# eora-ai/torchok

Measured on AMD Instinct MI355X. Metric: images/sec (node) ResNet-50 224px bs256/GPU; step p50 ms, higher is better.
Workload: dtype bf16

## Files before the change

### include/tok.h

```cpp
#ifndef TOK_H_
#define TOK_H_

#include <stddef.h>
#include <stdint.h>

#ifdef __cplusplus
extern "C" {
#endif

typedef enum tok_status {
  TOK_OK = 0,
  TOK_ERR_INVALID = -1,
  TOK_ERR_LAUNCH = -2,
  TOK_ERR_WORKSPACE = -3
} tok_status;

typedef enum tok_dtype { TOK_F32 = 0, TOK_F16 = 1, TOK_BF16 = 2 } tok_dtype;

typedef struct tok_conv_desc {
  int32_t n, h, w, c;
  int32_t k;
  int32_t r, s;
  int32_t p, q;
  int32_t stride, pad;
// ... 49 lines not shown
int tok_relu_mask_reduce(const void* dout, const uint8_t* mask, int64_t m, int c, void* dz, float* partial, void* stream);
int tok_bn3_bwd_prepare(const float* G, const float* w, const float* wz, const float* zsum, const float* partial, int rows,
                        int64_t count, int p, int k, const float* gamma, const float* mean, const float* rstd,
                        float* dgamma, float* dbeta, int param_accumulate, float* coef, float* dw, int dw_accumulate,
                        void* wa, void* wb, float* cvec, float* ws ,
                        void* stream);
size_t tok_bn3_bwd_prepare_ws_floats(int p, int k);
int tok_conv_dgrad_bias(const tok_conv_desc* d, const void* dy, const void* w_dgrad, const float* bias, void* dx,
                        int accumulate, const void* bn_y, const uint8_t* bn_mask, float* partial, void* stream);
int tok_subsample2_fwd(const void* x, int n, int h, int w, int c, void* out, void* stream);
int tok_subsample2_bwd(const void* dsub, int n, int h, int w, int c, void* dx, int accumulate, void* stream);
int tok_conv_dgrad_subacc_ok(const tok_conv_desc* d);
int tok_conv_dgrad_subacc(const tok_conv_desc* d, const void* dy, const void* w_dgrad, void* dx, const void* dsub,
                          const void* bn_y , const uint8_t* mask ,
                          float* partial , int mask_store, void* stream);
int tok_conv_dgrad2_ok(const tok_conv_desc* d1, const tok_conv_desc* d2);
int tok_conv_dgrad2(const tok_conv_desc* d1, const void* dy1, const void* w1_dgrad, const tok_conv_desc* d2, const void* dy2,
                    const void* w2_dgrad, const float* bias , void* dx, int accumulate,
                    const void* bn_y , const uint8_t* bn_mask , float* partial ,
                    void* stream);
size_t tok_conv_wgrad_ws_bytes(const tok_conv_desc* d);
int tok_conv_wgrad(const tok_conv_desc* d, const void* x, const void* dy, float* dw,
                   int k_real, int c_real, void* ws, size_t ws_bytes, int accumulate,
                   void* stream);
int tok_conv_wgrad_bias_ok(const tok_conv_desc* d);
size_t tok_conv_wgrad_bias_ws_bytes(const tok_conv_desc* d);
int tok_conv_wgrad_bias(const tok_conv_desc* d, const void* x, const void* dy, float* dw, int k_real, int c_real,
                        void* ws, size_t ws_bytes, int accumulate, float* dbias, int bias_accumulate, void* stream);


// ... 361 lines not shown
```

### torchok_amd/_C.py

```python
import ctypes
import os
from ctypes import POINTER, Structure, c_char_p, c_float, c_int, c_int32, c_int64, c_size_t, c_void_p

_HERE = os.path.dirname(os.path.abspath(__file__))
LIB_PATH = os.environ.get('TOK_LIB') or os.path.join(_HERE, 'lib', 'libtok_gfx950.so')

TOK_F32, TOK_F16, TOK_BF16 = 0, 1, 2
TOK_CE_LOSS_FLOATS = 2050


class ConvDesc(Structure):
    _fields_ = [('n', c_int32), ('h', c_int32), ('w', c_int32), ('c', c_int32),
                ('k', c_int32), ('r', c_int32), ('s', c_int32),
                ('p', c_int32), ('q', c_int32),
                ('stride', c_int32), ('pad', c_int32), ('s_pad', c_int32)]


class PackItem(Structure):
    _fields_ = [('src', c_void_p), ('dst_fwd', c_void_p), ('dst_dgrad', c_void_p),
                ('k', c_int32), ('r', c_int32), ('s', c_int32), ('c', c_int32),
                ('k_pad', c_int32), ('s_pad', c_int32), ('c_pad', c_int32), ('block_start', c_int32)]


TOK_GRAD_CLIP_MAX_PARTIALS = 1024
# ... 55 lines not shown
    'tok_colsum': (c_int, [_P, c_int64, c_int, c_int, _P, c_int, _P]),
    'tok_bn_gram_finalize': (c_int, [_P, _P, _P, c_int64, c_int, c_int, _P, _P, _P, _P, _P, c_float, c_float, _P, _P, _P, _P, _P, _P]),
    'tok_conv_fwd_bn_apply': (c_int, [POINTER(ConvDesc), _P, _P, _P, _P, _P, c_int, _P, _P, _P]),
    'tok_conv_dgrad_maskstore': (c_int, [POINTER(ConvDesc), _P, _P, _P, c_int, _P, _P, _P]),
    'tok_relu_mask_reduce': (c_int, [_P, _P, c_int64, c_int, _P, _P, _P]),
    'tok_bn3_bwd_prepare': (c_int, [_P, _P, _P, _P, _P, c_int, c_int64, c_int, c_int, _P, _P, _P, _P, _P, c_int, _P, _P, c_int,
                                    _P, _P, _P, _P, _P]),
    'tok_bn3_bwd_prepare_ws_floats': (c_size_t, [c_int, c_int]),
    'tok_conv_dgrad_bias': (c_int, [POINTER(ConvDesc), _P, _P, _P, _P, c_int, _P, _P, _P, _P]),
    'tok_conv_dgrad2_ok': (c_int, [POINTER(ConvDesc), POINTER(ConvDesc)]),
    'tok_conv_dgrad2': (c_int, [POINTER(ConvDesc), _P, _P, POINTER(ConvDesc), _P, _P, _P, _P, c_int, _P, _P, _P, _P]),
    'tok_subsample2_fwd': (c_int, [_P, c_int, c_int, c_int, c_int, _P, _P]),
    'tok_subsample2_bwd': (c_int, [_P, c_int, c_int, c_int, c_int, _P, c_int, _P]),
    'tok_conv_dgrad_subacc_ok': (c_int, [POINTER(ConvDesc)]),
    'tok_conv_dgrad_subacc': (c_int, [POINTER(ConvDesc), _P, _P, _P, _P, _P, _P, _P, c_int, _P]),
    'tok_softmax_ce_fwd': (c_int, [_P, _P, c_int, c_int, c_int, c_int64, _P, _P, _P, _P]),
    'tok_softmax_ce_bwd': (c_int, [_P, _P, _P, _P, _P, c_int, c_int, c_int, c_int64, _P, _P]),
    'tok_softmax_ce_smooth_fwd': (c_int, [_P, _P, c_int, c_int, c_int, c_int64, c_float, _P, _P, _P, _P]),
    'tok_softmax_ce_smooth_bwd': (c_int, [_P, _P, _P, _P, _P, c_int, c_int, c_int, c_int64, c_float, _P, _P]),
    'tok_upsample_ce_serves': (c_int, [c_int, c_int]),
    'tok_upsample_ce_fwd': (c_int, [_P, c_int, c_int, c_int, c_int, c_int, c_int, c_int, _P, c_int64, _P, _P, _P, _P]),
    'tok_upsample_ce_bwd': (c_int, [_P, c_int, c_int, c_int, c_int, c_int, c_int, c_int, _P, c_int64, _P, _P, _P, _P, c_int, _P]),
    'tok_dice_rows': (c_int, [c_int64]),
    'tok_dice_fwd': (c_int, [_P, _P, c_int64, c_int, c_int, c_int, c_float, c_float, c_int, _P, c_int, _P, _P, _P, _P]),
    'tok_dice_bwd': (c_int, [_P, _P, _P, _P, c_int64, c_int, c_int, c_int, _P, _P]),
    'tok_bce_logits_fwd': (c_int, [_P, _P, c_int64, c_int, c_int, c_float, c_int, _P, _P]),
    'tok_bce_logits_bwd': (c_int, [_P, _P, _P, _P, c_int64, c_int, c_int, c_float, c_int, _P, _P]),
    'tok_relevance_matrix_multilabel': (c_int, [_P, _P, c_int, c_int, c_int, _P, _P]),
    'tok_embed_reg_fwd': (c_int, [_P, c_int, c_int, c_int, c_int, _P, _P, _P]),
    'tok_embed_reg_bwd': (c_int, [_P, _P, _P, c_float, c_int, c_int, c_int, c_int, _P, _P]),
# ... 165 lines not shown
```

### torchok_amd/csrc/conv_common.h

```cpp
#pragma once
#include "tok_common.h"

struct FastDiv {
  uint32_t mul, shift;
};
static inline FastDiv make_fastdiv(uint32_t d) {
  FastDiv f;
  if (d <= 1) { f.mul = 0; f.shift = 0; return f; }
  uint32_t l = 0;
  while ((1ull << l) < d) ++l;
  f.mul = (uint32_t)((((1ull << 32) * ((1ull << l) - d)) / d) + 1);
  f.shift = l;
  return f;
}
__device__ __forceinline__ uint32_t fdiv(uint32_t n, FastDiv f) {
  return (uint32_t)(((uint64_t)__umulhi(n, f.mul) + n) >> f.shift);
}

struct ConvArgs {
  const bf16* x;
  const bf16* w;
  bf16* y;
  const float* bias;
  float* stats;
// ... 38 lines not shown
int conv_s2d_launch(ConvArgs& a, hipStream_t st);

bool gemm256_geometry(const ConvArgs& a);
bool gemm256_modes(const ConvArgs& a);
bool gemm256_serves(const ConvArgs& a);
int gemm256_rows(const ConvArgs& a);
void gemm256_tiles(const ConvArgs& a, int* gridM, int* gridN);
int gemm256_grid(int gridM, int gridN);
int gemm256_launch(ConvArgs& a, hipStream_t st);

bool stem_win_serves(const ConvArgs& a);
int stem_win_grid(const ConvArgs& a);
int stem_win_launch(ConvArgs& a, hipStream_t st);
bool stem_wgrad_serves(const tok_conv_desc* d);
int stem_wgrad_launch(const tok_conv_desc* d, const void* x, const void* dy, float* ws, int slabs, hipStream_t st);
```

### torchok_amd/csrc/conv_igemm.hip

```cpp
#include "conv_common.h"
#include "pw_gemm.h"
#include <stdlib.h>

namespace {

constexpr int BK = 64;
#ifdef TOK_NO_FRAG_ASM
constexpr bool FRAG_ASM = false;
#else
constexpr bool FRAG_ASM = true;
#endif
#ifdef TOK_NO_DMA
constexpr bool DMA_ENABLED = false;
#else
constexpr bool DMA_ENABLED = true;
#endif

__device__ __forceinline__ int fw_swz(int n) {
  return ((0x78 >> (((n >> 3) & 3) << 1)) & 3) | (((n >> 1) & 1) << 2);
}

template <int BM, int BN, int IN_DIV, bool C4, int PWM>
__global__ __launch_bounds__(256, (BN == 64 && PWM != 4) ? 3 : 2) void conv_igemm_kernel(ConvArgs a) {
  constexpr bool PW = PWM != 0;
// ... 691 lines not shown
  if (c4 && !m.bnep && stem_win_serves(a)) {
    r.kernel = K_STEM_WIN;
    r.grid = stem_win_grid(a);
    if (m.stats && r.grid > r.stat_rows) r.grid = r.stat_rows;
  }
  return r;
}

ConvRoute route_dgrad(const tok_conv_desc* d, const ConvArgs& a, ConvMode m) {
  if (d->stride == 1 && conv_win_serves(a)) return route_window(K_WIN, a);
  if (d->stride == 2 && conv_s2d_serves(a, d->stride, d->pad)) return route_window(K_S2D, a);
  const bool pointwise = d->r == 1 && d->s == 1 && d->stride == 1 && d->pad == 0;
  return route_gemm(a, pointwise, pick_bn(d->c, a.Ktot, d->h == 1 && d->w == 1), m);
}

int launch_ring(const ConvArgs& a, const ConvRoute& r, hipStream_t st) {
  PwArgs p = {};
  p.x = a.x; p.w = a.w; p.y = a.y; p.bias = a.bias; p.stats = a.stats;
  p.stat_rows = r.stat_rows;
  p.e1 = a.accumulate ? a.y : a.ep_short;
  p.e2 = a.bn_y; p.mask_in = a.bn_mask; p.mask_out = a.ep_mask;
  p.ep_scale = a.ep_scale; p.ep_shift = a.ep_shift; p.ep_relu = a.ep_relu;
  p.accumulate = a.accumulate; p.mask_store = a.mask_store;
  if (a.sub != nullptr) { p.e1 = a.sub; p.accumulate = 1; p.e1_sub = 1; p.sub_H = a.P; p.sub_W = a.Q; }
  p.M = a.M; p.C = a.C; p.N = a.K; p.gridM = r.gridM; p.gridN = r.gridN;
  return pw_ring_launch(p, r.bn_tile, r.grid, st);
}

template <int BN>
int launch_igemm(ConvArgs& a, int pw, int in_div, bool c4, hipStream_t st) {
  if (pw == 1) return launch_pw<128, BN, 1, false, 1>(a, st);
  if (pw == 3) return launch_pw<128, BN, 1, false, 3>(a, st);
  if (pw == 4) return launch_pw<128, BN, 1, false, 4>(a, st);
  if (c4) return launch_pw<128, BN, 1, true, 0>(a, st);
  return in_div == 2 ? launch_pw<128, BN, 2, false, 0>(a, st) : launch_pw<128, BN, 1, false, 0>(a, st);
}

int run_route(ConvArgs& a, const ConvRoute& r, int in_div, bool c4, hipStream_t st) {
  a.gridM = r.gridM; a.gridN = r.gridN; a.grid = r.grid; a.stat_rows = r.stat_rows;
  if (a.stats != nullptr) {
    const bool rows_agree = r.kernel == K_GEMM256 ? r.gridM <= r.stat_rows
// ... 218 lines not shown
  if (dgrad_fill(d, a)) return 0;
  return route_dgrad(d, a, ConvMode{false, false,  true, false}).kernel == K_RING ? 1 : 0;
}

extern "C" int tok_conv_dgrad_subacc(const tok_conv_desc* d, const void* dy, const void* w_dgrad, void* dx, const void* dsub,
                                     const void* bn_y, const uint8_t* mask, float* partial, int mask_store, void* stream) {
  TOK_CHECK_ARG(dsub != nullptr, "tok_conv_dgrad_subacc: dsub must not be null");
  TOK_CHECK_ARG(!mask_store || (mask && partial && !bn_y), "tok_conv_dgrad_subacc: mask_store needs mask + partial, no bn_y");
  TOK_CHECK_ARG(mask_store || ((bn_y == nullptr) == (partial == nullptr)), "tok_conv_dgrad_subacc: bn_y and partial go together");
  DgradEpilogue ep = {}; ep.bn_y = bn_y; ep.bn_mask = mask; ep.partial = partial; ep.mask_store = mask_store; ep.sub = dsub;
  return dgrad_impl(d, dy, w_dgrad, dx, ep, stream, "tok_conv_dgrad_subacc");
}


namespace {
bool dgrad2_route(const tok_conv_desc* d1, const tok_conv_desc* d2, ConvRoute* r) {
  if (d1 == nullptr || d2 == nullptr) return false;
  for (const tok_conv_desc* d : {d1, d2})
    if (!(d->r == 1 && d->s == 1 && d->stride == 1 && d->pad == 0 && d->k % 8 == 0 && d->c % 64 == 0)) return false;
  if (d1->n != d2->n || d1->h != d2->h || d1->w != d2->w || d1->c != d2->c) return false;
  const long long rows = (long long)d1->n * d1->h * d1->w;
  ConvArgs g = {};
  g.M = (int)rows; g.C = g.Ktot = d2->k; g.K = d2->c; g.R = g.S = g.stride = 1;
  g.gridM = tok_cdiv(rows, 128);
  *r = route_gemm(g, true, pick_bn(d2->c, d2->k), ConvMode{});
  return r->kernel == K_RING && r->bn_tile == 64;
}
}

extern "C" int tok_conv_dgrad2_ok(const tok_conv_desc* d1, const tok_conv_desc* d2) { ConvRoute r; return dgrad2_route(d1, d2, &r) ? 1 : 0; }
// ... 23 lines not shown
```

### torchok_amd/csrc/conv_wgrad.hip

```cpp
#include "tok_common.h"
#include "conv_common.h"
#include <type_traits>
#include <stdlib.h>

namespace {

struct WgradArgs {
  const bf16* x;
  const bf16* dy;
  float* ws;
  int H, W, C, K, R, S, P, Q, stride, pad;
  int M, PQ, HW, Ktot;
  int tilesN, tilesK, splitM, mchunk;
  uint32_t x_bytes, dy_bytes;
  uint32_t pq_mul, pq_shift, q_mul, q_shift;
  float* cs;
  int cs_cols;
  int adv_q, adv_p;
  size_t cs_stride, ws_stride;
};

__device__ __forceinline__ uint32_t magic_div(uint32_t n, uint32_t mul, uint32_t shift) {
  return (uint32_t)(((uint64_t)__umulhi(n, mul) + n) >> shift);
}
// ... 1135 lines not shown
    const size_t nb = (slab / 4 + 15) / 16;
    hipLaunchKernelGGL(wgrad_reduce_flat_kernel, dim3((int)(nb < 4096 ? nb : 4096)), dim3(256), 0, st,
                       (const float*)ws, dw, p.splitM, slab, accumulate, cs_inline ? a.ws_stride : slab,
                       cs_inline ? dbias : (float*)nullptr, k_real, cs_inline ? cs_pad : 0, bias_accumulate);
    TOK_CHECK_LAUNCH("tok_conv_wgrad(reduce)");
    return TOK_OK;
  }
  const size_t total = (size_t)k_real * d->r * d->s * c_real;
  const int blocks = (int)((total + 255) / 256 < 2048 ? (total + 255) / 256 : 2048);
  hipLaunchKernelGGL(wgrad_reduce_kernel, dim3(blocks), dim3(256), 0, st, (const float*)ws, dw,
                     p.splitM, k_real, d->r, d->s, c_real, d->k, d->s_pad, d->c, accumulate);
  TOK_CHECK_LAUNCH("tok_conv_wgrad(reduce)");
  return TOK_OK;
}
}
```

### torchok_amd/csrc/pw_gemm.h

```cpp
#pragma once
#include "tok_common.h"

struct PwArgs {
  const bf16* x;
  const bf16* w;
  bf16* y;
  const float* bias;
  float* stats;
  int stat_rows;
  const bf16* e1;
  const bf16* e2;
  const uint8_t* mask_in;
  uint8_t* mask_out;
  const float* ep_scale;
  const float* ep_shift;
  int ep_relu;
  int accumulate;
  int e1_sub, sub_H, sub_W;
  int mask_store;
  const bf16* x2;
  const bf16* w2;
  int C2;
  int M, C, N;
  int gridM, gridN;
};

int pw_ring_launch(const PwArgs& a, int bn_tile, int grid, hipStream_t st);
int pw_ring_grid(int bn_tile, int gridM, int gridN);
```

### torchok_amd/csrc/pw_gemm.hip

```cpp
#include "pw_gemm.h"
#include <stdlib.h>

namespace {

constexpr int BK = 64;
constexpr int BM = 128;

__device__ __forceinline__ int fw_swz(int n) {
  return ((0x78 >> (((n >> 3) & 3) << 1)) & 3) | (((n >> 1) & 1) << 2);
}

struct PwDiv { uint32_t mul, shift; };
PwDiv make_pwdiv(uint32_t d) {
  PwDiv f = {0, 0};
  if (d <= 1) return f;
  uint32_t l = 0;
  while ((1ull << l) < d) ++l;
  f.mul = (uint32_t)((((1ull << 32) * ((1ull << l) - d)) / d) + 1);
  f.shift = l;
  return f;
}
__device__ __forceinline__ uint32_t pwdiv(uint32_t n, PwDiv f) { return (uint32_t)(((uint64_t)__umulhi(n, f.mul) + n) >> f.shift); }

__device__ __forceinline__ u32x4 lds_read16(uint32_t addr) {
  u32x4 v;
  asm volatile("ds_read_b128 %0, %1" : "=v"(v) : "v"(addr));
  return v;
}
__device__ __forceinline__ uint32_t lds_read_u8(uint32_t addr) {
  uint32_t v;
  asm volatile("ds_read_u8 %0, %1" : "=v"(v) : "v"(addr));
  return v;
}

template <int BN, bool BNEP>
__global__ __launch_bounds__(256, BN == 64 ? 2 : 1) void pw_gemm_ring_kernel(PwArgs a, uint32_t x_bytes, uint32_t w_bytes,
                                                                             uint32_t y_bytes, uint32_t m_bytes, int KT,
                                                                             int SPT, uint32_t e1_bytes, PwDiv fd_hw, PwDiv fd_w,
                                                                             uint32_t x2_bytes, uint32_t w2_bytes, int KT1) {
  constexpr int NT = 256;
  constexpr int WGN = BN / 64;
  constexpr int WGM = (NT / 64) / WGN;
  constexpr int MT = BM / (WGM * 16);
  constexpr int RSTEP = NT / 8;
  constexpr int AROWS = BM / RSTEP;
  constexpr int WROWS = BN / RSTEP;
  constexpr int A_BYTES = BM * BK * 2;
  constexpr int W_BYTES = BN * BK * 2;
  constexpr int MK_BYTES = BN == 64 ? 1024 : 4096;
  constexpr int STAGE = A_BYTES + W_BYTES + MK_BYTES;
  constexpr int LOADS = AROWS + WROWS + 1;
  constexpr int NST = 3;

  extern __shared__ __attribute__((aligned(16))) char smem[];
// ... 8 lines not shown
  const int wm = wv / WGN;
  const int kc = tid & 7;
  const int lrow = tid >> 3;
  const int kcA = kc ^ (lrow & 7);
  const int kcW = kc ^ fw_swz(lrow);
  const int wave_u = __builtin_amdgcn_readfirstlane(tid >> 6);

  const __amdgpu_buffer_rsrc_t xsrd = __builtin_amdgcn_make_buffer_rsrc((void*)a.x, 0, x_bytes, 0x00020000);
  const __amdgpu_buffer_rsrc_t wsrd = __builtin_amdgcn_make_buffer_rsrc((void*)a.w, 0, w_bytes, 0x00020000);
  const __amdgpu_buffer_rsrc_t x2srd = __builtin_amdgcn_make_buffer_rsrc((void*)(a.x2 ? a.x2 : a.x), 0, a.x2 ? x2_bytes : 0, 0x00020000);
  const __amdgpu_buffer_rsrc_t w2srd = __builtin_amdgcn_make_buffer_rsrc((void*)(a.w2 ? a.w2 : a.w), 0, a.w2 ? w2_bytes : 0, 0x00020000);
  const __amdgpu_buffer_rsrc_t e1srd = __builtin_amdgcn_make_buffer_rsrc((void*)(a.e1 ? a.e1 : a.x), 0, a.e1 ? e1_bytes : 0, 0x00020000);
  const __amdgpu_buffer_rsrc_t e2srd = __builtin_amdgcn_make_buffer_rsrc((void*)(a.e2 ? a.e2 : a.x), 0, a.e2 ? y_bytes : 0, 0x00020000);
  const __amdgpu_buffer_rsrc_t msrd =
      __builtin_amdgcn_make_buffer_rsrc((void*)(a.mask_in ? (const void*)a.mask_in : (const void*)a.x), 0, a.mask_in ? m_bytes : 0, 0x00020000);

  const int xcd = blockIdx.x & 7, jx = blockIdx.x >> 3;
  const int bn_fixed = jx % a.gridN, jm = jx / a.gridN;
  const int S8 = (gridDim.x >> 3) / a.gridN;
  const int sweep = 8 * S8;
  const int n0 = bn_fixed * BN;
  const int it0 = xcd * S8 + jm;
  const int ntiles = it0 < a.gridM ? (a.gridM - it0 + sweep - 1) / sweep : 0;
  const int total = ntiles * SPT;
  const int nE1 = a.e1 != nullptr ? 1 : 0;
  const int mask_cols = a.N >> 3;

  int itL = it0, ksL = 0;
  auto issue = [&](int slot) {
    char* Adst = smem + slot * STAGE + wave_u * 1024;
    char* Wdst = smem + slot * STAGE + A_BYTES + wave_u * 1024;
    char* Mdst = smem + slot * STAGE + A_BYTES + W_BYTES + wave_u * (MK_BYTES / 4);
    const bool live = itL < a.gridM;
    const int m0 = itL * BM;
    const bool kstage = ksL < KT;
    const bool last = ksL == SPT - 1;
    if (kstage) {
      const bool second = ksL >= KT1;
      const int kl = second ? ksL - KT1 : ksL;
      const int Cc = second ? a.C2 : a.C;
      const __amdgpu_buffer_rsrc_t xs = second ? x2srd : xsrd;
      const __amdgpu_buffer_rsrc_t ws = second ? w2srd : wsrd;
      const int kcol = kl * BK + kcA * 8;
#pragma unroll
      for (int i = 0; i < AROWS; ++i) {
        const int m = m0 + lrow + RSTEP * i;
        uint32_t off = (live && m < a.M && kcol < Cc) ? (uint32_t)(m * Cc + kcol) * 2u : 0xFFFFFFF0u;
        asm volatile("" : "+v"(off));
        __builtin_amdgcn_raw_ptr_buffer_load_lds(xs, (lds_void*)(Adst + i * (RSTEP * 128)), 16, off, 0, 0, 0);
      }
      const int wcol = kl * BK + kcW * 8;
#pragma unroll
      for (int j = 0; j < WROWS; ++j) {
        const int n = n0 + lrow + RSTEP * j;
        uint32_t off = (live && n < a.N && wcol < Cc) ? (uint32_t)(n * Cc + wcol) * 2u : 0xFFFFFFF0u;
        asm volatile("" : "+v"(off));
        __builtin_amdgcn_raw_ptr_buffer_load_lds(ws, (lds_void*)(Wdst + j * (RSTEP * 128)), 16, off, 0, 0, 0);
      }
    } else {
      const bool first_e = (ksL - KT) == 0 && nE1;
      const __amdgpu_buffer_rsrc_t esrd = first_e ? e1srd : e2srd;
      const bool sub = first_e && a.e1_sub;
      auto erow = [&](int m, int n, bool ok) -> uint32_t {
        if (!ok) return 0xFFFFFFF0u;
        if (sub) {
          const uint32_t b = pwdiv((uint32_t)m, fd_hw);
          const uint32_t rem = (uint32_t)m - b * (uint32_t)(a.sub_H * a.sub_W);
          const uint32_t h = pwdiv(rem, fd_w);
          const uint32_t w = rem - h * (uint32_t)a.sub_W;
          if ((h | w) & 1u) return 0xFFFFFFF0u;
          const uint32_t ph = (uint32_t)(a.sub_H + 1) >> 1, pw = (uint32_t)(a.sub_W + 1) >> 1;
          return (((b * ph + (h >> 1)) * pw + (w >> 1)) * (uint32_t)a.N + (uint32_t)n) * 2u;
// ... 111 lines not shown
#pragma unroll
      for (int half = 0; half < 2; ++half) dst[mt][half] = __builtin_bit_cast(bf16x8, raw[mt][half]);
  };

  auto add_e1 = [&](uint32_t sb) {
    bf16x8 ev[MT][2];
    etile(sb, ev);
#pragma unroll
    for (int mt = 0; mt < MT; ++mt)
#pragma unroll
      for (int half = 0; half < 2; ++half)
#pragma unroll
        for (int e = 0; e < 8; ++e) acc[half * 2 + (e >> 2)][mt][e & 3] += bf2f(ev[mt][half][e]);
  };

  auto epilogue = [&](int it, uint32_t sb) {
    const int m0 = it * BM;
    const int nb = n0 + wn * 64 + sl * 8;
    bf16x8 ev[MT][2];
    const bool need_tile = BNEP ? (a.e1 != nullptr) : (a.e2 != nullptr);
    if (need_tile) etile(sb, ev);
    uint32_t mbits[MT][2];
    if (a.mask_in != nullptr) {
#pragma unroll
      for (int mt = 0; mt < MT; ++mt)
#pragma unroll
        for (int half = 0; half < 2; ++half)
          mbits[mt][half] = lds_read_u8(sb + A_BYTES + W_BYTES + (arow0 + mt * 16) * (BN / 8) + wn * 8 + sl + half * 4);
      asm volatile("s_waitcnt lgkmcnt(0)" ::: "memory");
      __builtin_amdgcn_sched_barrier(0);
    }
#pragma unroll
// ... 20 lines not shown
            if (a.ep_relu) z = fmaxf(z, 0.f);
            o[e] = f2bf(z);
            bits |= (bf2f(o[e]) > 0.f ? 1u : 0u) << e;
          }
          if (a.mask_out != nullptr) a.mask_out[eoff >> 3] = (uint8_t)bits;
        }
        if (a.mask_store) {
          const unsigned bits = mbits[mt][half];
#pragma unroll
          for (int e = 0; e < 8; ++e) {
            if (!((bits >> e) & 1u)) o[e] = (bf16)0.f;
            s1[half * 8 + e] += bf2f(o[e]);
          }
        }
        stg16(yp + half * 32, o);
        if (a.stats != nullptr && !a.mask_store) {
          if (a.e2 != nullptr) {
            const unsigned bits = a.mask_in != nullptr ? mbits[mt][half] : 0xffu;
#pragma unroll
            for (int e = 0; e < 8; ++e) {
              const float dz = ((bits >> e) & 1u) ? bf2f(o[e]) : 0.f;
              s1[half * 8 + e] += dz;
              s2[half * 8 + e] = fmaf(dz, bf2f(ev[mt][half][e]), s2[half * 8 + e]);
            }
          } else {
#pragma unroll
            for (int e = 0; e < 8; ++e) {
              const float r = bf2f(o[e]);
              s1[half * 8 + e] += r;
              s2[half * 8 + e] = fmaf(r, r, s2[half * 8 + e]);
            }
          }
        }
      }
    }
  };

  zero_acc();
  issue(0);
  issue(1);
  int cur = 0, nxt = 2;
  int itC = it0, ksC = 0;
  for (int s = 0; s < total; ++s) {
    asm volatile("s_waitcnt vmcnt(%0) lgkmcnt(0)" ::"n"(LOADS) : "memory");
    __builtin_amdgcn_s_barrier();
    issue(nxt);
    const uint32_t sb = lds_base + cur * STAGE;
    if (ksC < KT) {
      compute(sb);
    } else if (!BNEP && a.accumulate && ksC == KT) {
      add_e1(sb);
    }
    if (ksC == SPT - 1) {
      epilogue(itC, sb);
      zero_acc();
      ksC = 0;
      itC += sweep;
    } else {
      ++ksC;
    }
    cur = cur == NST - 1 ? 0 : cur + 1;
    nxt = nxt == NST - 1 ? 0 : nxt + 1;
  }
  asm volatile("s_waitcnt vmcnt(0) lgkmcnt(0)" ::: "memory");

  if (a.stats != nullptr) {
    __syncthreads();
    float* red = reinterpret_cast<float*>(smem);
#pragma unroll
    for (int step = 0; step < 4; ++step) {
      const int off = 8 >> step;
      const int cnt = 8 >> step;
      const bool up = (li & off) != 0;
#pragma unroll
      for (int j = 0; j < cnt; ++j) {
        const float send1 = up ? s1[j] : s1[j + cnt];
        const float send2 = up ? s2[j] : s2[j + cnt];
        const float keep1 = up ? s1[j + cnt] : s1[j];
        const float keep2 = up ? s2[j + cnt] : s2[j];
// ... 6 lines not shown
    red[(1 * WGM + wm) * BN + nl] = s2[0];
    __syncthreads();
    if (tid < 2 * BN) {
      const int which = tid / BN;
      const int c = tid - which * BN;
      float t = 0.f;
#pragma unroll
      for (int w_ = 0; w_ < WGM; ++w_) t += red[(which * WGM + w_) * BN + c];
      const int row = xcd * S8 + jm;
      const int n = n0 + c;
      if (n < a.N) a.stats[((size_t)which * a.stat_rows + row) * a.N + n] = t;
    }
  }
}

template <int BN, bool BNEP>
int launch_ring(const PwArgs& a, int grid, hipStream_t st) {
  constexpr int STAGE = BM * BK * 2 + BN * BK * 2 + (BN == 64 ? 1024 : 4096);
  constexpr int smem = 3 * STAGE;
  const int KT1 = tok_cdiv(a.C, BK);
  const int KT = KT1 + (a.x2 != nullptr ? tok_cdiv(a.C2, BK) : 0);
  const int SPT = KT + (a.e1 ? 1 : 0) + (a.e2 ? 1 : 0);
  const unsigned long long xb = (unsigned long long)a.M * a.C * 2, wb = (unsigned long long)a.N * a.C * 2,
                           yb = (unsigned long long)a.M * a.N * 2, mb = (unsigned long long)a.M * (a.N / 8);
  if (xb >= 0xFFFFFFF0ull || wb >= 0xFFFFFFF0ull || yb >= 0xFFFFFFF0ull) return 1;
  const unsigned long long x2b = a.x2 ? (unsigned long long)a.M * a.C2 * 2 : 0, w2b = a.x2 ? (unsigned long long)a.N * a.C2 * 2 : 0;
  if (x2b >= 0xFFFFFFF0ull) return 1;
  unsigned long long e1b = yb;
  PwDiv fd_hw = {0, 0}, fd_w = {0, 0};
  if (a.e1_sub) {
    const unsigned long long hw = (unsigned long long)a.sub_H * a.sub_W;
    e1b = (unsigned long long)(a.M / hw) * ((a.sub_H + 1) / 2) * ((a.sub_W + 1) / 2) * a.N * 2;
    fd_hw = make_pwdiv((uint32_t)hw);
    fd_w = make_pwdiv((uint32_t)a.sub_W);
  }
  tok_launch_lds<&pw_gemm_ring_kernel<BN, BNEP>>(smem, dim3(grid), dim3(256), smem, st, a, (uint32_t)xb, (uint32_t)wb, (uint32_t)yb,
                                                 (uint32_t)mb, KT, SPT, (uint32_t)e1b, fd_hw, fd_w, (uint32_t)x2b, (uint32_t)w2b, KT1);
  return 0;
}

}

int pw_ring_grid(int bn_tile, int gridM, int gridN) {
  const int unit = 8 * gridN;
  int G = 256 * (bn_tile == 64 ? 2 : 1);
  const long long need = (long long)gridM * gridN;
  if (need < G) G = (int)((need + unit - 1) / unit) * unit;
  G = G / unit * unit;
  if (G < unit) G = unit;
  return G;
}

int pw_ring_launch(const PwArgs& a, int bn_tile, int grid, hipStream_t st) {
  if (a.stats != nullptr && grid != a.stat_rows * a.gridN) return -1;
  if (a.C % 8 != 0 || a.N % 8 != 0) return 1;
  if (a.mask_in != nullptr && a.N % 64 != 0) return 1;
  if (a.accumulate && a.e1 == nullptr) return 1;
  if ((a.x2 == nullptr) != (a.w2 == nullptr) || (a.x2 != nullptr && (a.C2 <= 0 || a.C2 % 8 != 0))) return -1;
  if (a.e1_sub && (!a.accumulate || a.ep_scale != nullptr || a.sub_H <= 0 || a.sub_W <= 0 ||
                   a.M % (a.sub_H * a.sub_W) != 0)) return -1;
  const bool bnep = a.ep_scale != nullptr;
  if (bn_tile == 64) return bnep ? launch_ring<64, true>(a, grid, st) : launch_ring<64, false>(a, grid, st);
  if (bnep) return 1;
  return launch_ring<128, false>(a, grid, st);
}
```

### torchok_amd/engine/functional.py

```python
import weakref
from typing import Optional, Tuple

import os

import torch
from torch import nn

from .. import _C
from .core import _ms as _core_ms
from . import paramgrad as PG
from .core import BF16, Node, Region, TTensor, await_ready, donate_grad, grad_target, is_last_contribution, pad8, ptr, stream_ptr

F32 = torch.float32



class _Packs:
    __slots__ = ('fwd', 'dgrad', 'bias', 'key', 'synced', 'dims')

    def __init__(self):
        self.fwd = None
        self.dgrad = None
        self.bias = None
        self.key = None
# ... 360 lines not shown
            bs, bacc = PG.sink(conv.bias)
            PG.colsum(dy, m, kp, bs, bacc, two_pass=m > 4096 and kp == conv.bias.shape[0], n_real=conv.bias.shape[0])
            PG.commit(conv.bias, bs, bacc)
        if w_need:
            k, _, _, c = _krsc(conv.weight)
            PG.run_beside(self, side, (x.data, dy), raw_event=apply_event, fn=lambda: PG.weight_grad(
                d, x.data, dy, k, c, weight=conv.weight, bias=conv.bias if bias_in_wgrad else None)[1:])
        if x_need:
            prod = x.node
            rider = _dgrad_rider(x)
            sub = x.grad_sub if getattr(self, 'sub_capable', False) else None
            tgt, acc = grad_target(x, sub_ok=sub is not None)
            partial = _rider_partial(lib, rider, prod, d, x.cp, g.device)
            bn_y = ptr(prod.y) if rider == BN_SUMS else None
            bn_mask = ptr(prod.mask) if (rider == MASKED_DZ or (rider == BN_SUMS and prod.relu)) else None
            if sub is not None:
                x.grad_sub = None
                assert acc == 0
                _C.check(lib.tok_conv_dgrad_subacc(d, ptr(dy), ptr(self.pk.dgrad), ptr(tgt), ptr(sub), bn_y, bn_mask, ptr(partial),
                                                   int(rider == MASKED_DZ), st), 'tok_conv_dgrad_subacc')
            elif rider == MASKED_DZ:
                _C.check(lib.tok_conv_dgrad_maskstore(d, ptr(dy), ptr(self.pk.dgrad), ptr(tgt), acc, bn_mask, ptr(partial), st),
                         'tok_conv_dgrad_maskstore')
            elif rider == BN_SUMS:
                _C.check(lib.tok_conv_dgrad_bnstats(d, ptr(dy), ptr(self.pk.dgrad), ptr(tgt), acc, bn_y, bn_mask, ptr(partial), st),
                         'tok_conv_dgrad_bnstats')
            else:
                _C.check(lib.tok_conv_dgrad(d, ptr(dy), ptr(self.pk.dgrad), ptr(tgt), acc, st), 'tok_conv_dgrad')


BN_SUMS = 'bn_sums'
MASKED_DZ = 'masked_dz'


def _dgrad_rider(x: TTensor):
    prod = x.node
    if (isinstance(prod, _ConvBnActNode) and is_last_contribution(x) and prod.wants_fused_bwd_stats()
            and prod.fused_partial is None):
        return BN_SUMS
    if (isinstance(prod, _Unit3Node) and prod.relu and prod.mask is not None and is_last_contribution(x)
            and prod.masked_partial is None):
        return MASKED_DZ
    return None


def _rider_partial(lib, rider, prod, d, cp: int, dev) -> Optional[torch.Tensor]:
    if rider is None:
        return None
    rows = lib.tok_conv_dgrad_stat_rows(d)
    partial = torch.empty((2, rows, cp), dtype=F32, device=dev)
    if rider == MASKED_DZ:
        prod.masked_partial = (partial, rows)
    else:
        prod.fused_partial = (partial, rows)
    return partial



FUSE_UNIT3 = os.environ.get('TOK_FUSE_UNIT3', '1') != '0'
UNIT3_MIN_ROWS = int(os.environ.get('TOK_UNIT3_MIN_ROWS', '100000'))
# ... 5 lines not shown


def _colsum_f32(t: torch.Tensor, m: int, c: int) -> torch.Tensor:
    out = torch.empty(c, dtype=F32, device=t.device)
    PG.colsum(t, m, c, out, 0, two_pass=m > 4096, n_real=c)
    return out


class _Unit3Node(Node):
    needs_backward = True

    def __init__(self):
        self.x = self.out = self.shortcut = self.mask = None
        self.relu = True
        self.masked_partial = None

    def release(self):
        self.x = self.out = self.shortcut = self.mask = self.masked_partial = None
        self.mean = self.rstd = self.wz = self.zsum = self.pk = None

    def backward(self):
        lib, st = _C.lib(), stream_ptr()
        out: TTensor = self.out
        g = out.grad
        if g is None:
            return
        conv, bn, d, x, sc = self.conv, self.bn, self.desc, self.x, self.shortcut
        kp, p = d.k, d.c
        m = d.n * d.p * d.q
        dev = g.device
        if self.masked_partial is not None:
            partial, rows = self.masked_partial
            dz = g
# ... 5 lines not shown
                     'tok_relu_mask_reduce')
        out.grad = None
        if sc is not None and sc.requires_grad:
            if donate_grad(sc, dz):
                scn = sc.node
                if isinstance(scn, _Unit3Node) and not scn.relu and sc.uses == 1 and scn.masked_partial is None:
                    scn.masked_partial = (partial, rows)
            else:
                tgt, _ = grad_target(sc)
                tgt.add_(dz)
        w_need = conv.weight.requires_grad
        x_need = x.requires_grad
        g_need, b_need = bn.weight.requires_grad, bn.bias.requires_grad
        if not (w_need or x_need or g_need or b_need):
            return
        G = PG.weight_grad(d, x.data, dz, kp, p)[0]
        gbuf, bbuf, pacc, finish = PG.pair_sinks(bn.weight if g_need else None, bn.bias if b_need else None)
        dw, wacc = PG.sink(conv.weight) if w_need else (torch.empty((kp, p), dtype=F32, device=dev), 0)
        coef = torch.empty((3, kp), dtype=F32, device=dev)
        wa = torch.empty((p, kp), dtype=BF16, device=dev)
        wb = torch.empty((p, p), dtype=BF16, device=dev)
        cvec = torch.empty(p, dtype=F32, device=dev)
        scratch = torch.empty(lib.tok_bn3_bwd_prepare_ws_floats(p, kp), dtype=F32, device=dev)
        _C.check(lib.tok_bn3_bwd_prepare(ptr(G), ptr(conv.weight), ptr(self.wz), ptr(self.zsum), ptr(partial), rows, m, p,
                                         kp, ptr(bn.weight), ptr(self.mean), ptr(self.rstd), ptr(gbuf), ptr(bbuf), pacc,
                                         ptr(coef), ptr(dw), wacc, ptr(wa), ptr(wb), ptr(cvec), ptr(scratch), st),
                 'tok_bn3_bwd_prepare')
        finish()
        if w_need:
            PG.commit(conv.weight, dw, wacc)
        if not x_need:
# ... 725 lines not shown
```

Measured before the change: 14350.

## Fuse unit3 weight-gradient Gram computation into the preceding pointwise dgrad ring kernel

```diff
diff --git a/include/tok.h b/include/tok.h
--- a/include/tok.h
+++ b/include/tok.h
@@ -87,6 +87,11 @@
 int tok_conv_dgrad_subacc(const tok_conv_desc* d, const void* dy, const void* w_dgrad, void* dx, const void* dsub,
                           const void* bn_y , const uint8_t* mask ,
                           float* partial , int mask_store, void* stream);
+int tok_conv_dgrad_gram_ok(const tok_conv_desc* d, int p);
+size_t tok_conv_dgrad_gram_ws_bytes(const tok_conv_desc* d, int p);
+int tok_conv_dgrad_gram(const tok_conv_desc* d, const void* dy, const void* w_dgrad, void* dx, int accumulate,
+                        const void* dsub , const uint8_t* mask, float* partial, const void* gx, int p,
+                        void* ws, size_t ws_bytes, float* gram, void* stream);
 int tok_conv_dgrad2_ok(const tok_conv_desc* d1, const tok_conv_desc* d2);
 int tok_conv_dgrad2(const tok_conv_desc* d1, const void* dy1, const void* w1_dgrad, const tok_conv_desc* d2, const void* dy2,
                     const void* w2_dgrad, const float* bias , void* dx, int accumulate,
diff --git a/torchok_amd/_C.py b/torchok_amd/_C.py
--- a/torchok_amd/_C.py
+++ b/torchok_amd/_C.py
@@ -93,6 +93,9 @@
     'tok_subsample2_bwd': (c_int, [_P, c_int, c_int, c_int, c_int, _P, c_int, _P]),
     'tok_conv_dgrad_subacc_ok': (c_int, [POINTER(ConvDesc)]),
     'tok_conv_dgrad_subacc': (c_int, [POINTER(ConvDesc), _P, _P, _P, _P, _P, _P, _P, c_int, _P]),
+    'tok_conv_dgrad_gram_ok': (c_int, [POINTER(ConvDesc), c_int]),
+    'tok_conv_dgrad_gram_ws_bytes': (c_size_t, [POINTER(ConvDesc), c_int]),
+    'tok_conv_dgrad_gram': (c_int, [POINTER(ConvDesc), _P, _P, _P, c_int, _P, _P, _P, _P, c_int, _P, c_size_t, _P, _P]),
     'tok_softmax_ce_fwd': (c_int, [_P, _P, c_int, c_int, c_int, c_int64, _P, _P, _P, _P]),
     'tok_softmax_ce_bwd': (c_int, [_P, _P, _P, _P, _P, c_int, c_int, c_int, c_int64, _P, _P]),
     'tok_softmax_ce_smooth_fwd': (c_int, [_P, _P, c_int, c_int, c_int, c_int64, c_float, _P, _P, _P, _P]),
diff --git a/torchok_amd/csrc/conv_common.h b/torchok_amd/csrc/conv_common.h
--- a/torchok_amd/csrc/conv_common.h
+++ b/torchok_amd/csrc/conv_common.h
@@ -76,3 +76,5 @@
 int stem_win_launch(ConvArgs& a, hipStream_t st);
 bool stem_wgrad_serves(const tok_conv_desc* d);
 int stem_wgrad_launch(const tok_conv_desc* d, const void* x, const void* dy, float* ws, int slabs, hipStream_t st);
+
+void wgrad_fold_slabs(const float* ws, float* out, int slabs, size_t slab, hipStream_t st);
diff --git a/torchok_amd/csrc/conv_igemm.hip b/torchok_amd/csrc/conv_igemm.hip
--- a/torchok_amd/csrc/conv_igemm.hip
+++ b/torchok_amd/csrc/conv_igemm.hip
@@ -729,7 +729,7 @@
   return route_gemm(a, pointwise, pick_bn(d->c, a.Ktot, d->h == 1 && d->w == 1), m);
 }
 
-int launch_ring(const ConvArgs& a, const ConvRoute& r, hipStream_t st) {
+int launch_ring(const ConvArgs& a, const ConvRoute& r, hipStream_t st, const PwGram* gram = nullptr) {
   PwArgs p = {};
   p.x = a.x; p.w = a.w; p.y = a.y; p.bias = a.bias; p.stats = a.stats;
   p.stat_rows = r.stat_rows;
@@ -739,7 +739,7 @@
   p.accumulate = a.accumulate; p.mask_store = a.mask_store;
   if (a.sub != nullptr) { p.e1 = a.sub; p.accumulate = 1; p.e1_sub = 1; p.sub_H = a.P; p.sub_W = a.Q; }
   p.M = a.M; p.C = a.C; p.N = a.K; p.gridM = r.gridM; p.gridN = r.gridN;
-  return pw_ring_launch(p, r.bn_tile, r.grid, st);
+  return pw_ring_launch(p, r.bn_tile, r.grid, st, gram);
 }
 
 template <int BN>
@@ -988,6 +988,56 @@
 
 
 namespace {
+bool dgrad_gram_route(const tok_conv_desc* d, int p, ConvArgs& a, ConvRoute* r) {
+  if (check_desc(d, "tok_conv_dgrad_gram")) return false;
+  if (!(d->r == 1 && d->s == 1 && d->stride == 1 && d->pad == 0 && d->c % 8 == 0)) return false;
+  if (p != 64 && p != 128) return false;
+  if (dgrad_fill(d, a)) return false;
+  if ((unsigned long long)a.M * p * 2 >= 0xFFFFFFF0ull) return false;
+  *r = route_dgrad(d, a, ConvMode{false, false, false, true});
+  return r->kernel == K_RING && r->bn_tile == 64;
+}
+}
+
+extern "C" int tok_conv_dgrad_gram_ok(const tok_conv_desc* d, int p) {
+  ConvArgs a = {};
+  ConvRoute r;
+  return dgrad_gram_route(d, p, a, &r) ? 1 : 0;
+}
+
+extern "C" size_t tok_conv_dgrad_gram_ws_bytes(const tok_conv_desc* d, int p) {
+  ConvArgs a = {};
+  ConvRoute r;
+  if (!dgrad_gram_route(d, p, a, &r)) return 0;
+  return (size_t)r.stat_rows * d->c * p * sizeof(float);
+}
+
+extern "C" int tok_conv_dgrad_gram(const tok_conv_desc* d, const void* dy, const void* w_dgrad, void* dx, int accumulate,
+                                   const void* dsub, const uint8_t* mask, float* partial, const void* gx, int p, void* ws,
+                                   size_t ws_bytes, float* gram, void* stream) {
+  ConvArgs a = {};
+  ConvRoute r;
+  TOK_CHECK_ARG(dgrad_gram_route(d, p, a, &r), "tok_conv_dgrad_gram: layer / width not served (ask tok_conv_dgrad_gram_ok)");
+  TOK_CHECK_ARG(dy && w_dgrad && dx && mask && partial && gx && ws && gram, "tok_conv_dgrad_gram: null pointer");
+  TOK_CHECK_ARG(dsub == nullptr || !accumulate, "tok_conv_dgrad_gram: dsub already is the accumulate stage");
+  TOK_CHECK_ARG(ws_bytes >= tok_conv_dgrad_gram_ws_bytes(d, p), "tok_conv_dgrad_gram: workspace too small");
+  TOK_CHECK_ARG((((uintptr_t)ws | (uintptr_t)gram) & 15) == 0, "tok_conv_dgrad_gram: ws / gram must be 16-byte aligned");
+  a.x = (const bf16*)dy; a.w = (const bf16*)w_dgrad; a.y = (bf16*)dx;
+  a.stats = partial; a.bn_mask = mask; a.mask_store = 1; a.accumulate = accumulate; a.sub = (const bf16*)dsub;
+  a.gridM = r.gridM; a.gridN = r.gridN; a.grid = r.grid; a.stat_rows = r.stat_rows;
+  PwGram g = {};
+  g.x = (const bf16*)gx; g.slab = (float*)ws; g.P = p;
+  hipStream_t st = tok_stream(stream);
+  const int rc = launch_ring(a, r, st, &g);
+  if (rc != 0) { tok_set_error("tok_conv_dgrad_gram: ring kernel refused the launch (%d)", rc); return TOK_ERR_INVALID; }
+  TOK_CHECK_LAUNCH("tok_conv_dgrad_gram");
+  wgrad_fold_slabs((const float*)ws, gram, r.stat_rows, (size_t)d->c * p, st);
+  TOK_CHECK_LAUNCH("tok_conv_dgrad_gram(fold)");
+  return TOK_OK;
+}
+
+
+namespace {
 bool dgrad2_route(const tok_conv_desc* d1, const tok_conv_desc* d2, ConvRoute* r) {
   if (d1 == nullptr || d2 == nullptr) return false;
   for (const tok_conv_desc* d : {d1, d2})
diff --git a/torchok_amd/csrc/conv_wgrad.hip b/torchok_amd/csrc/conv_wgrad.hip
--- a/torchok_amd/csrc/conv_wgrad.hip
+++ b/torchok_amd/csrc/conv_wgrad.hip
@@ -1173,3 +1173,9 @@
   return TOK_OK;
 }
 }
+
+void wgrad_fold_slabs(const float* ws, float* out, int slabs, size_t slab, hipStream_t st) {
+  const size_t nb = (slab / 4 + 15) / 16;
+  hipLaunchKernelGGL(wgrad_reduce_flat_kernel, dim3((int)(nb < 4096 ? nb : 4096)), dim3(256), 0, st, ws, out, slabs, slab, 0, slab,
+                     (float*)nullptr, 0, 0, 0);
+}
diff --git a/torchok_amd/csrc/pw_gemm.h b/torchok_amd/csrc/pw_gemm.h
--- a/torchok_amd/csrc/pw_gemm.h
+++ b/torchok_amd/csrc/pw_gemm.h
@@ -25,5 +25,12 @@
   int gridM, gridN;
 };
 
-int pw_ring_launch(const PwArgs& a, int bn_tile, int grid, hipStream_t st);
+struct PwGram {
+  const bf16* x;
+  float* slab;
+  uint32_t x_bytes;
+  int P;
+};
+
+int pw_ring_launch(const PwArgs& a, int bn_tile, int grid, hipStream_t st, const PwGram* gram = nullptr);
 int pw_ring_grid(int bn_tile, int gridM, int gridN);
diff --git a/torchok_amd/csrc/pw_gemm.hip b/torchok_amd/csrc/pw_gemm.hip
--- a/torchok_amd/csrc/pw_gemm.hip
+++ b/torchok_amd/csrc/pw_gemm.hip
@@ -33,11 +33,22 @@
   return v;
 }
 
-template <int BN, bool BNEP>
+__device__ __forceinline__ u32x2 lds_read_tr(uint32_t addr) {
+  u32x2 v;
+  asm volatile("ds_read_b64_tr_b16 %0, %1" : "=v"(v) : "v"(addr));
+  return v;
+}
+__device__ __forceinline__ void lds_write16(uint32_t addr, u32x4 v) {
+  asm volatile("ds_write_b128 %0, %1" ::"v"(addr), "v"(v) : "memory");
+}
+
+template <int BN, bool BNEP, int PG>
 __global__ __launch_bounds__(256, BN == 64 ? 2 : 1) void pw_gemm_ring_kernel(PwArgs a, uint32_t x_bytes, uint32_t w_bytes,
                                                                              uint32_t y_bytes, uint32_t m_bytes, int KT,
                                                                              int SPT, uint32_t e1_bytes, PwDiv fd_hw, PwDiv fd_w,
-                                                                             uint32_t x2_bytes, uint32_t w2_bytes, int KT1) {
+                                                                             uint32_t x2_bytes, uint32_t w2_bytes, int KT1,
+                                                                             PwGram gr) {
+  static_assert(PG == 0 || (BN == 64 && !BNEP), "Gram rider: 64-wide tiles, no BatchNorm epilogue");
   constexpr int NT = 256;
   constexpr int WGN = BN / 64;
   constexpr int WGM = (NT / 64) / WGN;
@@ -76,6 +87,7 @@
   const __amdgpu_buffer_rsrc_t e2srd = __builtin_amdgcn_make_buffer_rsrc((void*)(a.e2 ? a.e2 : a.x), 0, a.e2 ? y_bytes : 0, 0x00020000);
   const __amdgpu_buffer_rsrc_t msrd =
       __builtin_amdgcn_make_buffer_rsrc((void*)(a.mask_in ? (const void*)a.mask_in : (const void*)a.x), 0, a.mask_in ? m_bytes : 0, 0x00020000);
+  const __amdgpu_buffer_rsrc_t gxsrd = __builtin_amdgcn_make_buffer_rsrc((void*)(PG > 0 ? gr.x : a.x), 0, PG > 0 ? gr.x_bytes : 0, 0x00020000);
 
   const int xcd = blockIdx.x & 7, jx = blockIdx.x >> 3;
   const int bn_fixed = jx % a.gridN, jm = jx / a.gridN;
@@ -87,6 +99,7 @@
   const int total = ntiles * SPT;
   const int nE1 = a.e1 != nullptr ? 1 : 0;
   const int mask_cols = a.N >> 3;
+  const int ksE = SPT - (PG > 0 ? PG : 1);
 
   int itL = it0, ksL = 0;
   auto issue = [&](int slot) {
@@ -96,7 +109,8 @@
     const bool live = itL < a.gridM;
     const int m0 = itL * BM;
     const bool kstage = ksL < KT;
-    const bool last = ksL == SPT - 1;
+    const bool last = ksL == ksE;
+    const bool gstage = PG > 0 && ksL >= ksE;
     if (kstage) {
       const bool second = ksL >= KT1;
       const int kl = second ? ksL - KT1 : ksL;
@@ -118,6 +132,21 @@
         uint32_t off = (live && n < a.N && wcol < Cc) ? (uint32_t)(n * Cc + wcol) * 2u : 0xFFFFFFF0u;
         asm volatile("" : "+v"(off));
         __builtin_amdgcn_raw_ptr_buffer_load_lds(ws, (lds_void*)(Wdst + j * (RSTEP * 128)), 16, off, 0, 0, 0);
+      }
+    } else if (gstage) {
+      const int kcol = (ksL - ksE) * BK + kcA * 8;
+#pragma unroll
+      for (int i = 0; i < AROWS; ++i) {
+        const int m = m0 + lrow + RSTEP * i;
+        uint32_t off = (live && m < a.M) ? (uint32_t)(m * gr.P + kcol) * 2u : 0xFFFFFFF0u;
+        asm volatile("" : "+v"(off));
+        __builtin_amdgcn_raw_ptr_buffer_load_lds(gxsrd, (lds_void*)(Adst + i * (RSTEP * 128)), 16, off, 0, 0, 0);
+      }
+#pragma unroll
+      for (int j = 0; j < WROWS; ++j) {
+        uint32_t off = 0xFFFFFFF0u;
+        asm volatile("" : "+v"(off));
+        __builtin_amdgcn_raw_ptr_buffer_load_lds(gxsrd, (lds_void*)(Wdst + j * (RSTEP * 128)), 16, off, 0, 0, 0);
       }
     } else {
       const bool first_e = (ksL - KT) == 0 && nE1;
@@ -259,8 +288,19 @@
         for (int e = 0; e < 8; ++e) acc[half * 2 + (e >> 2)][mt][e & 3] += bf2f(ev[mt][half][e]);
   };
 
+  u32x4 og[MT][2];
+  f32x4 gacc[PG > 0 ? 4 * PG : 1];
+#pragma unroll
+  for (int t = 0; t < (PG > 0 ? 4 * PG : 1); ++t) gacc[t] = (f32x4){0.f, 0.f, 0.f, 0.f};
+
   auto epilogue = [&](int it, uint32_t sb) {
     const int m0 = it * BM;
+    if constexpr (PG > 0) {
+#pragma unroll
+      for (int mt = 0; mt < MT; ++mt)
+#pragma unroll
+        for (int half = 0; half < 2; ++half) og[mt][half] = (u32x4){0u, 0u, 0u, 0u};
+    }
     const int nb = n0 + wn * 64 + sl * 8;
     bf16x8 ev[MT][2];
     const bool need_tile = BNEP ? (a.e1 != nullptr) : (a.e2 != nullptr);
@@ -311,6 +351,7 @@
           }
         }
         stg16(yp + half * 32, o);
+        if constexpr (PG > 0) og[mt][half] = __builtin_bit_cast(u32x4, o);
         if (a.stats != nullptr && !a.mask_store) {
           if (a.e2 != nullptr) {
             const unsigned bits = a.mask_in != nullptr ? mbits[mt][half] : 0xffu;
@@ -330,6 +371,51 @@
           }
         }
       }
+    }
+  };
+
+  auto gram = [&](uint32_t sb, int g) {
+    const uint32_t Xb = sb, Db = sb + A_BYTES;
+    const int q = li >> 2, p = li & 3;
+    const int r7 = (4 * sl + q) & 7;
+#pragma unroll
+    for (int h = 0; h < 2; ++h) {
+      if ((wave_u >> 1) == h) {
+#pragma unroll
+        for (int mt = 0; mt < MT; ++mt)
+#pragma unroll
+          for (int half = 0; half < 2; ++half) {
+            const int r = (wave_u & 1) * 32 + mt * 16 + li;
+            lds_write16(Db + r * 128 + (((sl + 4 * half) ^ (r & 7)) << 4), og[mt][half]);
+          }
+      }
+      asm volatile("s_waitcnt lgkmcnt(0)" ::: "memory");
+      __builtin_amdgcn_s_barrier();
+#pragma unroll
+      for (int ks = 0; ks < 2; ++ks) {
+        u32x2 df[2], xf[4][2];
+#pragma unroll
+        for (int u = 0; u < 2; ++u) {
+          const int R = 32 * ks + 16 * u + 4 * sl + q;
+          df[u] = lds_read_tr(Db + R * 128 + (((2 * wv + (p >> 1)) ^ r7) << 4) + 8 * (p & 1));
+#pragma unroll
+          for (int pt = 0; pt < 4; ++pt)
+            xf[pt][u] = lds_read_tr(Xb + (64 * h + R) * 128 + (((2 * pt + (p >> 1)) ^ r7) << 4) + 8 * (p & 1));
+        }
+        asm volatile("s_waitcnt lgkmcnt(0)" ::: "memory");
+        __builtin_amdgcn_sched_barrier(0);
+        const u32x4 dv = {df[0][0], df[0][1], df[1][0], df[1][1]};
+#pragma unroll
+        for (int pt = 0; pt < 4; ++pt) {
+          const u32x4 xv = {xf[pt][0][0], xf[pt][0][1], xf[pt][1][0], xf[pt][1][1]};
+#pragma unroll
+          for (int gg = 0; gg < (PG > 0 ? PG : 1); ++gg)
+            if (gg == g)
+              gacc[4 * gg + pt] = __builtin_amdgcn_mfma_f32_16x16x32_bf16(__builtin_bit_cast(bf16x8, dv), __builtin_bit_cast(bf16x8, xv),
+                                                                          gacc[4 * gg + pt], 0, 0, 0);
+        }
+      }
+      if (h == 0) __builtin_amdgcn_s_barrier();
     }
   };
 
@@ -348,18 +434,40 @@
     } else if (!BNEP && a.accumulate && ksC == KT) {
       add_e1(sb);
     }
-    if (ksC == SPT - 1) {
-      epilogue(itC, sb);
-      zero_acc();
-      ksC = 0;
-      itC += sweep;
+    if constexpr (PG == 0) {
+      if (ksC == SPT - 1) {
+        epilogue(itC, sb);
+        zero_acc();
+        ksC = 0;
+        itC += sweep;
+      } else {
+        ++ksC;
+      }
     } else {
-      ++ksC;
+      if (ksC == ksE) {
+        epilogue(itC, sb);
+        zero_acc();
+      }
+      if (ksC >= ksE) gram(sb, ksC - ksE);
+      if (ksC == SPT - 1) {
+        ksC = 0;
+        itC += sweep;
+      } else {
+        ++ksC;
+      }
     }
     cur = cur == NST - 1 ? 0 : cur + 1;
     nxt = nxt == NST - 1 ? 0 : nxt + 1;
   }
   asm volatile("s_waitcnt vmcnt(0) lgkmcnt(0)" ::: "memory");
+
+  if constexpr (PG > 0) {
+    float* gb = gr.slab + ((size_t)(xcd * S8 + jm) * a.N + n0 + 16 * wv + 4 * sl) * gr.P + li;
+#pragma unroll
+    for (int t = 0; t < 4 * PG; ++t)
+#pragma unroll
+      for (int r = 0; r < 4; ++r) gb[(size_t)r * gr.P + 16 * t] = gacc[t][r];
+  }
 
   if (a.stats != nullptr) {
     __syncthreads();
@@ -396,13 +504,13 @@
   }
 }
 
-template <int BN, bool BNEP>
-int launch_ring(const PwArgs& a, int grid, hipStream_t st) {
+template <int BN, bool BNEP, int PG>
+int launch_ring(const PwArgs& a, int grid, hipStream_t st, const PwGram& gr = PwGram{}) {
   constexpr int STAGE = BM * BK * 2 + BN * BK * 2 + (BN == 64 ? 1024 : 4096);
   constexpr int smem = 3 * STAGE;
   const int KT1 = tok_cdiv(a.C, BK);
   const int KT = KT1 + (a.x2 != nullptr ? tok_cdiv(a.C2, BK) : 0);
-  const int SPT = KT + (a.e1 ? 1 : 0) + (a.e2 ? 1 : 0);
+  const int SPT = KT + (a.e1 ? 1 : 0) + (a.e2 ? 1 : 0) + PG;
   const unsigned long long xb = (unsigned long long)a.M * a.C * 2, wb = (unsigned long long)a.N * a.C * 2,
                            yb = (unsigned long long)a.M * a.N * 2, mb = (unsigned long long)a.M * (a.N / 8);
   if (xb >= 0xFFFFFFF0ull || wb >= 0xFFFFFFF0ull || yb >= 0xFFFFFFF0ull) return 1;
@@ -416,8 +524,9 @@
     fd_hw = make_pwdiv((uint32_t)hw);
     fd_w = make_pwdiv((uint32_t)a.sub_W);
   }
-  tok_launch_lds<&pw_gemm_ring_kernel<BN, BNEP>>(smem, dim3(grid), dim3(256), smem, st, a, (uint32_t)xb, (uint32_t)wb, (uint32_t)yb,
-                                                 (uint32_t)mb, KT, SPT, (uint32_t)e1b, fd_hw, fd_w, (uint32_t)x2b, (uint32_t)w2b, KT1);
+  tok_launch_lds<&pw_gemm_ring_kernel<BN, BNEP, PG>>(smem, dim3(grid), dim3(256), smem, st, a, (uint32_t)xb, (uint32_t)wb, (uint32_t)yb,
+                                                     (uint32_t)mb, KT, SPT, (uint32_t)e1b, fd_hw, fd_w, (uint32_t)x2b, (uint32_t)w2b, KT1,
+                                                     gr);
   return 0;
 }
 
@@ -433,8 +542,13 @@
   return G;
 }
 
-int pw_ring_launch(const PwArgs& a, int bn_tile, int grid, hipStream_t st) {
+int pw_ring_launch(const PwArgs& a, int bn_tile, int grid, hipStream_t st, const PwGram* gram) {
   if (a.stats != nullptr && grid != a.stat_rows * a.gridN) return -1;
+  if (gram != nullptr) {
+    if (bn_tile != 64 || !a.mask_store || a.stats == nullptr || a.mask_in == nullptr || a.e2 != nullptr || a.x2 != nullptr ||
+        a.ep_scale != nullptr || gram->x == nullptr || gram->slab == nullptr || (gram->P != 64 && gram->P != 128)) return -1;
+    if ((unsigned long long)a.M * gram->P * 2 >= 0xFFFFFFF0ull) return 1;
+  }
   if (a.C % 8 != 0 || a.N % 8 != 0) return 1;
   if (a.mask_in != nullptr && a.N % 64 != 0) return 1;
   if (a.accumulate && a.e1 == nullptr) return 1;
@@ -442,7 +556,12 @@
   if (a.e1_sub && (!a.accumulate || a.ep_scale != nullptr || a.sub_H <= 0 || a.sub_W <= 0 ||
                    a.M % (a.sub_H * a.sub_W) != 0)) return -1;
   const bool bnep = a.ep_scale != nullptr;
-  if (bn_tile == 64) return bnep ? launch_ring<64, true>(a, grid, st) : launch_ring<64, false>(a, grid, st);
+  if (gram != nullptr) {
+    PwGram g = *gram;
+    g.x_bytes = (uint32_t)((unsigned long long)a.M * g.P * 2);
+    return g.P == 64 ? launch_ring<64, false, 1>(a, grid, st, g) : launch_ring<64, false, 2>(a, grid, st, g);
+  }
+  if (bn_tile == 64) return bnep ? launch_ring<64, true, 0>(a, grid, st) : launch_ring<64, false, 0>(a, grid, st);
   if (bnep) return 1;
-  return launch_ring<128, false>(a, grid, st);
-}
+  return launch_ring<128, false, 0>(a, grid, st);
+}
diff --git a/torchok_amd/engine/functional.py b/torchok_amd/engine/functional.py
--- a/torchok_amd/engine/functional.py
+++ b/torchok_amd/engine/functional.py
@@ -398,7 +398,17 @@
             partial = _rider_partial(lib, rider, prod, d, x.cp, g.device)
             bn_y = ptr(prod.y) if rider == BN_SUMS else None
             bn_mask = ptr(prod.mask) if (rider == MASKED_DZ or (rider == BN_SUMS and prod.relu)) else None
-            if sub is not None:
+            if rider == MASKED_DZ and _gram_rides(lib, prod, d):
+                gp = prod.desc.c
+                assert sub is None or acc == 0
+                if sub is not None:
+                    x.grad_sub = None
+                wsb = lib.tok_conv_dgrad_gram_ws_bytes(d, gp)
+                ws = torch.empty(wsb // 4, dtype=F32, device=g.device)
+                prod.gram = torch.empty((x.cp, gp), dtype=F32, device=g.device)
+                _C.check(lib.tok_conv_dgrad_gram(d, ptr(dy), ptr(self.pk.dgrad), ptr(tgt), acc, ptr(sub), bn_mask, ptr(partial),
+                                                 ptr(prod.x.data), gp, ptr(ws), wsb, ptr(prod.gram), st), 'tok_conv_dgrad_gram')
+            elif sub is not None:
                 x.grad_sub = None
                 assert acc == 0
                 _C.check(lib.tok_conv_dgrad_subacc(d, ptr(dy), ptr(self.pk.dgrad), ptr(tgt), ptr(sub), bn_y, bn_mask, ptr(partial),
@@ -428,6 +438,18 @@
     return None
 
 
+GRAM_RIDER_MAX_P = 64
+
+
+def _gram_rides(lib, prod, d) -> bool:
+    ok = getattr(lib, 'tok_conv_dgrad_gram_ok', None)
+    if ok is None or prod.desc.c > GRAM_RIDER_MAX_P:
+        return False
+    conv, bn = prod.conv, prod.bn
+    wanted = conv.weight.requires_grad or prod.x.requires_grad or bn.weight.requires_grad or bn.bias.requires_grad
+    return bool(wanted and ok(d, prod.desc.c))
+
+
 def _rider_partial(lib, rider, prod, d, cp: int, dev) -> Optional[torch.Tensor]:
     if rider is None:
         return None
@@ -463,9 +485,10 @@
         self.x = self.out = self.shortcut = self.mask = None
         self.relu = True
         self.masked_partial = None
+        self.gram = None
 
     def release(self):
-        self.x = self.out = self.shortcut = self.mask = self.masked_partial = None
+        self.x = self.out = self.shortcut = self.mask = self.masked_partial = self.gram = None
         self.mean = self.rstd = self.wz = self.zsum = self.pk = None
 
     def backward(self):
@@ -501,7 +524,7 @@
         g_need, b_need = bn.weight.requires_grad, bn.bias.requires_grad
         if not (w_need or x_need or g_need or b_need):
             return
-        G = PG.weight_grad(d, x.data, dz, kp, p)[0]
+        G = self.gram if self.gram is not None else PG.weight_grad(d, x.data, dz, kp, p)[0]
         gbuf, bbuf, pacc, finish = PG.pair_sinks(bn.weight if g_need else None, bn.bias if b_need else None)
         dw, wacc = PG.sink(conv.weight) if w_need else (torch.empty((kp, p), dtype=F32, device=dev), 0)
         coef = torch.empty((3, kp), dtype=F32, device=dev)
```

Result: no change. 14470, median of 6 (+0.9%).
